# Sienna12321/MSHA--GNN

Measured on AMD Instinct MI355X. Metric: edges/sec GAT fwd+bwd @1 GPU; link-score pairs/sec; achieved HBM GB/s vs peak, higher is better.
Workload: dtype f32; 1 GPU; gat_layer_syn100k; nodes=100000, cols=100000, edges=2000000, in_features=128, heads=8, feat=16, parallelism=replicas1

## Files before the change

### msha--gnn_amd/csrc/edge_attention.hip

```cpp
#include <stdlib.h>

#include <cstdlib>

#include "common.h"
#include "edge_geo.h"

#ifndef COLS_EH
#define COLS_EH 1
#endif
#ifndef DE_SLOT_MIN_BYTES
#define DE_SLOT_MIN_BYTES (192ll << 20)
#endif
#ifndef COLS_WIDE_UG
#define COLS_WIDE_UG 4
#endif
#ifndef COLS_EPI_BUF
#define COLS_EPI_BUF 1
#endif
#ifndef COLS_NARROW_UG
#define COLS_NARROW_UG 8
#endif
#ifndef COLS_NG
#define COLS_NG 2
#endif

namespace msha {

template <int H, int F, typename T, int EPL>
__global__ void __launch_bounds__(256) edge_attn_fwd_kernel(
    const int32_t* __restrict__ rowptr, const int32_t* __restrict__ col,
    const uint8_t* __restrict__ rowflag, int64_t n_rows, const float* __restrict__ el,
    const float* __restrict__ er, const T* __restrict__ hc, float slope, Dropout dp,
    T* __restrict__ u, T* __restrict__ u_lo, float* __restrict__ lse, float* __restrict__ attd) {
  using G = Geo<H, F, T>;
  constexpr int CEL = EPL * G::CE;
  const int lane = lane_id();
  const int e_s = lane / H, h_s = lane % H;
  const int g_e = G::QPL == 1 ? lane / G::NQ : 0;
  const int64_t wave = ((int64_t)blockIdx.x * blockDim.x + threadIdx.x) >> 6;
  const int64_t nwaves = ((int64_t)gridDim.x * blockDim.x) >> 6;

  int64_t row = wave;
  if (row >= n_rows) return;
  int32_t start = rowptr[row], end = rowptr[row + 1];
  bool virt = rowflag != nullptr && rowflag[row] != 0;
  float elh = el[row * H + h_s];
  int32_t j0[EPL], j1[EPL];
#pragma unroll
  for (int t = 0; t < EPL; ++t) {
    const int32_t e0 = start + t * G::CE + e_s, e1 = e0 + CEL;
    j0[t] = e0 < end ? col[e0] : 0;
    j1[t] = e1 < end ? col[e1] : 0;
  }
  while (true) {
    const int64_t nrow = row + nwaves;
    const bool has_next = nrow < n_rows;
    const int32_t nstart = has_next ? rowptr[nrow] : 0;
    const int32_t nend = has_next ? rowptr[nrow + 1] : 0;
    float m = -INFINITY, l = 0.f;
    Pk<T> acc[G::QPL];
#pragma unroll
    for (int k = 0; k < G::QPL; ++k) acc[k] = pk_zero<T>();
    float erv[EPL];
#pragma unroll
    for (int t = 0; t < EPL; ++t)
      erv[t] = start + t * G::CE + e_s < end ? er[(int64_t)j0[t] * H + h_s] : 0.f;

    for (int32_t cs = start; cs < end; cs += CEL) {
      int32_t j[EPL], j2[EPL];
      float ern[EPL], sc[EPL];
      bool valid[EPL];
      float smax = -INFINITY;
#pragma unroll
      for (int t = 0; t < EPL; ++t) {
        const int32_t e = cs + t * G::CE + e_s;
        valid[t] = e < end;
        j[t] = j0[t];
        j2[t] = e + 2 * CEL < end ? col[e + 2 * CEL] : 0;
        ern[t] = e + CEL < end ? er[(int64_t)j1[t] * H + h_s] : 0.f;
        sc[t] = valid[t] ? (virt ? 0.f : lrelu(elh + erv[t], slope)) : -INFINITY;
        smax = fmaxf(smax, sc[t]);
      }
      const float mn = fmaxf(m, wave_xor_max<H>(smax));
      const float alpha = __expf(m - mn);
      float w[EPL], psum = 0.f;
#pragma unroll
      for (int t = 0; t < EPL; ++t) {
        const float pe = valid[t] ? __expf(sc[t] - mn) : 0.f;
        psum += pe;
        w[t] = valid[t] ? pe * dropout_factor(dp, (uint64_t)(cs + t * G::CE + e_s) * H + h_s)
                        : 0.f;
      }
      l = fmaf(l, alpha, wave_xor_sum<H>(psum));
      m = mn;
#pragma unroll
      for (int k = 0; k < G::QPL; ++k) {
        const int hd = quad_of<G>(lane, k) / G::QH;
        acc[k] = pk_scale(acc[k], __shfl(alpha, hd));
      }
      const int nvalid = min(CEL, (int)(end - cs));
#pragma unroll
      for (int g = 0; g < CEL; g += G::EPI) {
        if (g >= nvalid) break;
        const int t = g / G::CE;
        const int ei = g % G::CE + g_e;
        const int32_t jq = __shfl(j[t], ei * H);
// ... 479 lines not shown
        }
      }
    }
    if (G::EPI > 1) {
#pragma unroll
      for (int o = G::NQ; o < 64; o <<= 1) acc[0] = pk_xor_add(acc[0], o);
    }
#pragma unroll
    for (int k = 0; k < G::QPL; ++k) {
      if (g_e != 0) continue;
      const int q = quad_of<G>(lane, k);
      if (whole) {
        pk_store(out + (int64_t)jc * G::D + G::V * q, acc[k]);
      } else {
        float* dst = part + c * G::D + G::V * q;
#pragma unroll
        for (int i = 0; i < G::V; i += 4)
          *reinterpret_cast<float4*>(dst + i) =
              make_float4(acc[k].v[i], acc[k].v[i + 1], acc[k].v[i + 2], acc[k].v[i + 3]);
      }
    }
    if (HASX) {
      xacc = wave_xor_sum<H>(xacc);
      if (lane < H) (whole ? out_x + (int64_t)jc * H : part_x + c * H)[lane] = xacc;
    }
  }
}

constexpr int kCombineWaves = 16;

template <typename T>
__global__ void __launch_bounds__(1024) csc_combine_kernel(
    const int32_t* __restrict__ multi_col, const int32_t* __restrict__ multi_first,
    const int32_t* __restrict__ multi_count, int64_t n_multi, int D, int H,
    const float* __restrict__ part, const float* __restrict__ part_x, T* __restrict__ out,
    float* __restrict__ out_x) {
  __shared__ float red[kCombineWaves][256];
  const int W = D + (part_x != nullptr ? H : 0);
  const int64_t mi = blockIdx.x;
  const int e0 = blockIdx.y * 256;
  const int lane = threadIdx.x & 63, g = threadIdx.x >> 6;
  const int32_t jc = multi_col[mi], first = multi_first[mi], cnt = multi_count[mi];
  float acc[4] = {0.f, 0.f, 0.f, 0.f};
  auto ld = [&](int64_t c, int q) {
    const int e = e0 + lane + 64 * q;
    return e < D ? part[c * D + e] : (e < W ? part_x[c * H + (e - D)] : 0.f);
  };
  int k = g;
  for (; k + 3 * kCombineWaves < cnt; k += 4 * kCombineWaves) {
    float v[4][4];
#pragma unroll
    for (int u = 0; u < 4; ++u)
#pragma unroll
      for (int q = 0; q < 4; ++q) v[u][q] = ld(first + k + u * kCombineWaves, q);
#pragma unroll
    for (int u = 0; u < 4; ++u)
#pragma unroll
      for (int q = 0; q < 4; ++q) acc[q] += v[u][q];
  }
  for (; k < cnt; k += kCombineWaves) {
#pragma unroll
    for (int q = 0; q < 4; ++q) acc[q] += ld(first + k, q);
  }
#pragma unroll
  for (int q = 0; q < 4; ++q) red[g][lane + 64 * q] = acc[q];
  __syncthreads();
  for (int w = kCombineWaves / 2; w >= 1; w >>= 1) {
    if (g < w) {
#pragma unroll
      for (int q = 0; q < 4; ++q) red[g][lane + 64 * q] += red[g + w][lane + 64 * q];
    }
    __syncthreads();
  }
  if (g == 0) {
#pragma unroll
    for (int q = 0; q < 4; ++q) {
      const int e = e0 + lane + 64 * q;
      if (e < D) out[(int64_t)jc * D + e] = from_f32<T>(red[0][lane + 64 * q]);
      else if (e < W) out_x[(int64_t)jc * H + (e - D)] = red[0][lane + 64 * q];
    }
  }
}

#ifndef REC_PAD
#define REC_PAD 1
#endif
__host__ __device__ constexpr int rec_stride(int H) {
  int s = 1;
  while (s < 3 * H) s <<= 1;
  return REC_PAD ? s : 3 * H;
}
__host__ __device__ constexpr bool rec_has_flag(int H) { return rec_stride(H) > 3 * H; }

template <int H, int F, typename T, bool RT = false>
__global__ void __launch_bounds__(256) bwd_row_stats_kernel(
    int64_t n_rows, const float* __restrict__ el, const float* __restrict__ lse,
    const T* __restrict__ u, const T* __restrict__ u_lo, const T* __restrict__ dU,
    float* __restrict__ rec, const float* __restrict__ uc, const float* __restrict__ qc,
    const uint8_t* __restrict__ rowflag, float* __restrict__ d_el) {
  using G = Geo<H, F, T>;
  constexpr int UNR = G::QPL == 1 ? 4 : 1;
  constexpr int RPW = G::EPI * UNR;
  const int lane = lane_id();
  const int r_s = G::QPL == 1 ? lane / G::NQ : 0;
  const int64_t wave = ((int64_t)blockIdx.x * blockDim.x + threadIdx.x) >> 6;
  const int64_t nwaves = ((int64_t)gridDim.x * blockDim.x) >> 6;
  for (int64_t r0 = wave * RPW; r0 < n_rows; r0 += nwaves * RPW) {
    Pk<T> a[UNR][G::QPL], b[UNR][G::QPL];
    float4 c[UNR][G::QPL][RT ? G::V / 4 : 1];
    float elv[UNR][G::QPL], lsev[UNR][G::QPL], qcv[UNR][G::QPL];
    uint8_t fl[UNR];
    const bool lo = sizeof(T) == 2 && u_lo != nullptr;
#pragma unroll
    for (int g = 0; g < UNR; ++g) {
      const int64_t row = min(r0 + g * G::EPI + r_s, n_rows - 1);
#pragma unroll
      for (int k = 0; k < G::QPL; ++k) {
        const int q = quad_of<G>(lane, k);
        a[g][k] = pk_load(dU + row * G::D + G::V * q);
        b[g][k] = pk_load(u + row * G::D + G::V * q);
      }
#pragma unroll
      for (int k = 0; k < G::QPL; ++k) {
        const int q = quad_of<G>(lane, k);
        if (RT) {
#pragma unroll
          for (int v = 0; v < G::V / 4; ++v)
            c[g][k][v] = *reinterpret_cast<const float4*>(uc + row * G::D + G::V * q + 4 * v);
          qcv[g][k] = qc[row * H + q / G::QH];
        }
        elv[g][k] = el[row * H + q / G::QH];
        lsev[g][k] = lse[row * H + q / G::QH];
      }
      fl[g] = rowflag != nullptr ? rowflag[row] : (uint8_t)0;
    }
#pragma unroll
    for (int g = 0; g < UNR; ++g) {
      const int64_t row = r0 + g * G::EPI + r_s;
#pragma unroll
      for (int k = 0; k < G::QPL; ++k) {
        const int q = quad_of<G>(lane, k);
        float dot = pk_dot(a[g][k], b[g][k]);
        if (lo) {
          const int64_t rr = min(row, n_rows - 1);
          dot += pk_dot(a[g][k], pk_load(u_lo + rr * G::D + G::V * q));
        }
        const float dk = group_sum<G::QH>(dot);
        float dc = 0.f;
        if (RT) {
          float cv = 0.f;
#pragma unroll
          for (int v = G::V - 4; v >= 0; v -= 4) {
            const float4 c4 = c[g][k][v / 4];
            cv = fmaf(a[g][k].v[v + 3], c4.w, cv);
            cv = fmaf(a[g][k].v[v + 2], c4.z, cv);
            cv = fmaf(a[g][k].v[v + 1], c4.y, cv);
            cv = fmaf(a[g][k].v[v], c4.x, cv);
          }
          dc = group_sum<G::QH>(cv);
        }
        if (q % G::QH == 0 && row < n_rows) {
          const int h = q / G::QH;
          float* r = rec + row * rec_stride(H);
          r[h] = elv[g][k];
          r[H + h] = lsev[g][k];
          r[2 * H + h] = dk;
          const bool virt = fl[g] != 0;
          if (rec_has_flag(H) && h == 0) r[3 * H] = virt ? 1.f : 0.f;
          if (RT) d_el[row * H + h] = virt ? 0.f : fmaf(-dk, qcv[g][k], dc);
        }
      }
    }
  }
}

template <int H, int F, typename T, bool BUF, bool RSC = false>
__global__ void __launch_bounds__(256) bwd_cols_kernel(
    const int32_t* __restrict__ chunk_col, const int32_t* __restrict__ chunk_start,
    const int32_t* __restrict__ chunk_end, int64_t n_chunks, const int32_t* __restrict__ colptr,
    const int32_t* __restrict__ csc_row, const int32_t* __restrict__ csc_eid, int64_t n_rows,
    const uint8_t* __restrict__ rowflag, const float* __restrict__ rec,
    const float* __restrict__ er, const float* __restrict__ ar, const T* __restrict__ hc,
    const T* __restrict__ dU, float slope, Dropout dp, bool slot_de, float* __restrict__ de,
    T* __restrict__ d_hc, float* __restrict__ d_er, float* __restrict__ part,
    float* __restrict__ part_x) {
  using G = Geo<H, F, T>;
  const int lane = lane_id();
  const int e_s = lane / H, h_s = lane % H;
  const int g_e = G::QPL == 1 ? lane / G::NQ : 0;
  const int dsrc_k = (h_s * G::QH) / 64;
  const int dsrc_l = (h_s * G::QH) % 64;
  const int64_t wave = ((int64_t)blockIdx.x * blockDim.x + threadIdx.x) >> 6;
  const int64_t nwaves = ((int64_t)gridDim.x * blockDim.x) >> 6;

  int64_t c = wave;
  if (c >= n_chunks) return;
  int32_t jc = chunk_col[c], s0 = chunk_start[c], s1 = chunk_end[c];
  int32_t i0 = s0 + e_s < s1 ? csc_row[s0 + e_s] : 0;
  int32_t i1 = s0 + G::CE + e_s < s1 ? csc_row[s0 + G::CE + e_s] : 0;
  while (true) {
    const int64_t nc = c + nwaves;
    const bool has_next = nc < n_chunks;
    const int32_t njc = has_next ? chunk_col[nc] : 0;
    const int32_t ns0 = has_next ? chunk_start[nc] : 0;
    const int32_t ns1 = has_next ? chunk_end[nc] : 0;
    const bool whole = s0 == colptr[jc] && s1 == colptr[jc + 1];
    Pk<T> hcq[G::QPL], acc[G::QPL];
#pragma unroll
    for (int k = 0; k < G::QPL; ++k) {
      hcq[k] = pk_load(hc + (int64_t)jc * G::D + G::V * quad_of<G>(lane, k));
      acc[k] = pk_zero<T>();
    }
    float erh;
    if (RSC && G::QPL == 1) {
      const int q = lane % G::NQ;
      Pk<T> aq;
#pragma unroll
      for (int v = 0; v < G::V; ++v) aq.v[v] = ar[G::V * q + v];
      erh = __shfl(group_sum<G::QH>(pk_dot(hcq[0], aq)), h_s * G::QH);
    } else {
      erh = er[(int64_t)jc * H + h_s];
    }
    float xacc = 0.f;
    for (int32_t cs = s0; cs < s1; cs += G::CE) {
      const int32_t slot = cs + e_s;
      const bool valid = slot < s1;
      const int32_t i = i0;
      const int64_t eid = valid ? (int64_t)csc_eid[slot] : 0;
      float pre = 0.f, att = 0.f, dropf = 0.f, Dsi = 0.f;
      bool virt = false;
      if (valid) {
        const float* r = rec + (int64_t)i * rec_stride(H);
        virt = rowflag != nullptr && rowflag[i] != 0;
        pre = r[h_s] + erh;
        const float sv = virt ? 0.f : lrelu(pre, slope);
        att = __expf(sv - r[H + h_s]);
        Dsi = r[2 * H + h_s];
        dropf = dropout_factor(dp, (uint64_t)eid * H + h_s);
      }
      const float wv = att * dropf;
      const int nvalid = min(G::CE, (int)(s1 - cs));
      float gsum = 0.f;
      if constexpr (BUF && (G::EPI == 1 || COLS_EPI_BUF)) {
        constexpr int UG = G::EPI == 1 ? COLS_WIDE_UG : COLS_NARROW_UG;
        const rsrc_t r_dU = make_rsrc(dU, (uint32_t)(n_rows * G::D * sizeof(T)));
#pragma unroll
        for (int g0 = 0; g0 < G::CE; g0 += UG * G::EPI) {
          if (g0 >= nvalid) break;
          u32x4_t dl[UG][G::QPL];
#pragma unroll
          for (int u = 0; u < UG; ++u) {
            const int g = g0 + u * G::EPI;
            if (g >= G::CE) break;
            const int ei = g + g_e;
            const int32_t iq = __shfl(i, ei * H);
#pragma unroll
            for (int k = 0; k < G::QPL; ++k) {
              const int q = quad_of<G>(lane, k);
              const uint32_t off = ei < nvalid
                  ? (uint32_t)iq * (uint32_t)(G::D * sizeof(T)) + (uint32_t)(G::V * q * sizeof(T))
                  : kOOB;
              dl[u][k] = buf_b128(r_dU, off);
            }
          }
#pragma unroll
          for (int u = 0; u < UG; ++u) {
            const int g = g0 + u * G::EPI;
            if (g >= G::CE || g >= nvalid) break;
            const int ei = g + g_e;
            const bool mine = e_s >= g && e_s < g + G::EPI;
            const int srcl =
                G::QPL == 1 ? ((e_s - g) & (G::EPI - 1)) * G::NQ + h_s * G::QH : dsrc_l;
#pragma unroll
            for (int k = 0; k < G::QPL; ++k) {
              const int q = quad_of<G>(lane, k);
              const float wq = __shfl(wv, ei * H + q / G::QH);
              const Pk<T> dUi = pk_from_raw(dl[u][k], (T*)nullptr);
              acc[k] = pk_fma(wq, dUi, acc[k]);
              float t = pk_dot(dUi, hcq[k]);
              t = group_sum<G::QH>(t);
              const float cand = __shfl(t, srcl);
              if (mine && (G::QPL == 1 || k == dsrc_k)) gsum = cand;
            }
          }
        }
      } else {
#pragma unroll
      for (int g = 0; g < G::CE; g += G::EPI) {
        if (g >= nvalid) break;
        const int ei = g + g_e;
        const int32_t iq = __shfl(i, ei * H);
        const bool mine = e_s >= g && e_s < g + G::EPI;
        const int srcl = G::QPL == 1 ? ((e_s - g) & (G::EPI - 1)) * G::NQ + h_s * G::QH : dsrc_l;
#pragma unroll
        for (int k = 0; k < G::QPL; ++k) {
          const int q = quad_of<G>(lane, k);
          const float wq = __shfl(wv, ei * H + q / G::QH);
          float t = 0.f;
          if (ei < nvalid) {
            const Pk<T> dUi = pk_load(dU + (int64_t)iq * G::D + G::V * q);
            acc[k] = pk_fma(wq, dUi, acc[k]);
            t = pk_dot(dUi, hcq[k]);
          }
          t = group_sum<G::QH>(t);
          const float cand = __shfl(t, srcl);
          if (mine && (G::QPL == 1 || k == dsrc_k)) gsum = cand;
        }
      }
      }
      const int32_t sl2 = slot + 2 * G::CE;
      const int32_t i2 = sl2 < s1 ? csc_row[sl2] : 0;
      if (valid) {
        const float ds = att * (gsum * dropf - Dsi);
        const float dev = virt ? 0.f : ds * (pre > 0.f ? 1.f : slope);
        if (de != nullptr) de[(slot_de ? (int64_t)slot : eid) * H + h_s] = dev;
        xacc += dev;
      }
      i0 = i1;
      i1 = i2;
    }
    if (has_next) {
      const int32_t a0 = ns0 + e_s, a1 = ns0 + G::CE + e_s;
      i0 = a0 < ns1 ? csc_row[a0] : 0;
      i1 = a1 < ns1 ? csc_row[a1] : 0;
    }
    if (G::EPI > 1) {
#pragma unroll
      for (int o = G::NQ; o < 64; o <<= 1) acc[0] = pk_xor_add(acc[0], o);
    }
#pragma unroll
    for (int k = 0; k < G::QPL; ++k) {
      if (g_e != 0) continue;
      const int q = quad_of<G>(lane, k);
      if (whole) {
        pk_store(d_hc + (int64_t)jc * G::D + G::V * q, acc[k]);
      } else {
        float* dst = part + c * G::D + G::V * q;
#pragma unroll
        for (int v = 0; v < G::V; v += 4)
          *reinterpret_cast<float4*>(dst + v) =
              make_float4(acc[k].v[v], acc[k].v[v + 1], acc[k].v[v + 2], acc[k].v[v + 3]);
      }
    }
    xacc = wave_xor_sum<H>(xacc);
    if (lane < H) (whole ? d_er + (int64_t)jc * H : part_x + c * H)[lane] = xacc;
    if (!has_next) break;
    c = nc;
    jc = njc;
    s0 = ns0;
    s1 = ns1;
  }
}

template <int H, int F, typename T, bool RSC = false>
__global__ void __launch_bounds__(256) bwd_cols_eh_kernel(
    const int32_t* __restrict__ chunk_col, const int32_t* __restrict__ chunk_start,
    const int32_t* __restrict__ chunk_end, int64_t n_chunks, const int32_t* __restrict__ colptr,
    const int32_t* __restrict__ csc_row, const int32_t* __restrict__ csc_eid, int64_t n_edges,
    const uint8_t* __restrict__ rowflag, int64_t n_rows, const float* __restrict__ rec,
    const float* __restrict__ er, const float* __restrict__ ar, const T* __restrict__ hc,
    const T* __restrict__ dU, float slope, Dropout dp, bool slot_de, float* __restrict__ de,
    T* __restrict__ d_hc, float* __restrict__ d_er, float* __restrict__ part,
    float* __restrict__ part_x) {
  using G = Geo<H, F, T>;
  constexpr int NV = G::QH;
  constexpr int NG = COLS_NG;
  const int lane = lane_id();
  const int e_s = lane / H, h_s = lane % H;
  const int64_t wave = ((int64_t)blockIdx.x * blockDim.x + threadIdx.x) >> 6;
  const int64_t nwaves = ((int64_t)gridDim.x * blockDim.x) >> 6;
  const rsrc_t r_row = make_rsrc(csc_row, (uint32_t)(n_edges * 4));
  const rsrc_t r_eid = make_rsrc(csc_eid, (uint32_t)(n_edges * 4));
  const rsrc_t r_flag = make_rsrc(rowflag, (uint32_t)n_rows);
  const rsrc_t r_rec = make_rsrc(rec, (uint32_t)(n_rows * 4 * rec_stride(H)));
  const rsrc_t r_dU = make_rsrc(dU, (uint32_t)(n_rows * G::D * sizeof(T)));
  const rsrc_t r_de = make_rsrc(de, (uint32_t)(n_edges * 4 * H));
  const uint32_t h_off = h_s * F * sizeof(T);
  const bool need_eid = dp.active || (de != nullptr && !slot_de);

  int64_t c = wave;
  if (c >= n_chunks) return;
  int32_t jc = chunk_col[c], s0 = chunk_start[c], s1 = chunk_end[c];
  int32_t ii[NG];
#pragma unroll
  for (int g = 0; g < NG; ++g) {
    const int32_t a = s0 + g * G::CE + e_s;
    ii[g] = buf_i32(r_row, a < s1 ? (uint32_t)a * 4u : kOOB);
  }
  while (true) {
    const int64_t nc = c + nwaves;
    const bool has_next = nc < n_chunks;
    const int32_t njc = has_next ? chunk_col[nc] : 0;
    const int32_t ns0 = has_next ? chunk_start[nc] : 0;
    const int32_t ns1 = has_next ? chunk_end[nc] : 0;
    const bool whole = s0 == colptr[jc] && s1 == colptr[jc + 1];
    Pk<T> hcv[NV], acc[NV];
#pragma unroll
    for (int k = 0; k < NV; ++k) {
      hcv[k] = pk_load(hc + (int64_t)jc * G::D + h_s * F + G::V * k);
      acc[k] = pk_zero<T>();
    }
    const float er_tab = RSC ? 0.f : er[(int64_t)jc * H + h_s];
    float xacc = 0.f;
    for (int32_t cs = s0; cs < s1; cs += NG * G::CE) {
      Pk<T> dUv[NG][NV];
      int32_t eid[NG];
      float r_el[NG], r_lse[NG], Dsi[NG];
      uint32_t vflag[NG];
#pragma unroll
      for (int g = 0; g < NG; ++g) {
        const bool valid = cs + g * G::CE + e_s < s1;
        const uint32_t row_off = valid ? (uint32_t)ii[g] * (G::D * sizeof(T)) + h_off : kOOB;
#pragma unroll
        for (int k = 0; k < NV; ++k)
          dUv[g][k] = pk_load_buf(r_dU, row_off + (valid ? k * 16u : 0u), (T*)nullptr);
        eid[g] = buf_i32(r_eid, valid && need_eid ? (uint32_t)(cs + g * G::CE + e_s) * 4u : kOOB);
        const uint32_t rec_off = valid ? (uint32_t)ii[g] * (4u * rec_stride(H)) + h_s * 4u : kOOB;
        r_el[g] = buf_f32(r_rec, rec_off);
        r_lse[g] = buf_f32(r_rec, valid ? rec_off + 4u * H : kOOB);
        Dsi[g] = buf_f32(r_rec, valid ? rec_off + 8u * H : kOOB);
        if constexpr (rec_has_flag(H))
          vflag[g] = __float_as_uint(buf_f32(r_rec, valid ? rec_off - h_s * 4u + 12u * H : kOOB));
        else
          vflag[g] = buf_u8(r_flag, valid ? (uint32_t)ii[g] : kOOB);
      }
#pragma unroll
      for (int g = 0; g < NG; ++g) {
        const int32_t a = cs + (NG + g) * G::CE + e_s;
        ii[g] = buf_i32(r_row, a < s1 ? (uint32_t)a * 4u : kOOB);
      }
      float erh = er_tab;
      if (RSC) {
        Pk<T> hv[NV];
#pragma unroll
        for (int k = 0; k < NV; ++k) {
          hv[k] = hcv[k];
#pragma unroll
          for (int v = 0; v < G::V; ++v) asm volatile("" : "+v"(hv[k].v[v]));
        }
        erh = head_score<NV>(hv, ar + h_s * F);
      }
#pragma unroll
      for (int g = 0; g < NG; ++g) {
        const int32_t slot = cs + g * G::CE + e_s;
        const bool valid = slot < s1;
        const bool virt = vflag[g] != 0;
        const float pre = r_el[g] + erh;
        const float sv = virt ? 0.f : lrelu(pre, slope);
        const float att = __expf(sv - r_lse[g]);
        const float dropf = dropout_factor(dp, (uint64_t)eid[g] * H + h_s);
        const float wv = valid ? att * dropf : 0.f;
        float d[NV];
#pragma unroll
        for (int k = 0; k < NV; ++k) {
          d[k] = pk_dot(dUv[g][k], hcv[k]);
          acc[k] = pk_fma(wv, dUv[g][k], acc[k]);
        }
#pragma unroll
        for (int o = 1; o < NV; o <<= 1)
#pragma unroll
          for (int k = 0; k < NV; k += 2 * o) d[k] = d[k] + d[k + o];
        const float ds = att * (d[0] * dropf - Dsi[g]);
        const float dev = virt ? 0.f : ds * (pre > 0.f ? 1.f : slope);
#ifndef DIAG_NO_DE
        const uint32_t at = slot_de ? (uint32_t)slot : (uint32_t)eid[g];
        buf_store_f32(r_de, valid ? at * (4u * H) + h_s * 4u : kOOB, dev);
#endif
        xacc += valid ? dev : 0.f;
      }
    }
#pragma unroll
    for (int g = 0; g < NG; ++g) {
      const int32_t a = ns0 + g * G::CE + e_s;
      ii[g] = buf_i32(r_row, a < ns1 ? (uint32_t)a * 4u : kOOB);
    }
#pragma unroll
    for (int k = 0; k < NV; ++k)
#pragma unroll
      for (int o = H; o < 64; o <<= 1) acc[k] = pk_xor_add(acc[k], o);
    if (e_s == 0) {
#pragma unroll
      for (int k = 0; k < NV; ++k) {
        if (whole) {
          pk_store(d_hc + (int64_t)jc * G::D + h_s * F + G::V * k, acc[k]);
        } else {
          float* dst = part + c * G::D + h_s * F + G::V * k;
#pragma unroll
          for (int v = 0; v < G::V; v += 4)
            *reinterpret_cast<float4*>(dst + v) =
                make_float4(acc[k].v[v], acc[k].v[v + 1], acc[k].v[v + 2], acc[k].v[v + 3]);
        }
      }
    }
    xacc = wave_xor_sum<H>(xacc);
    if (lane < H) (whole ? d_er + (int64_t)jc * H : part_x + c * H)[lane] = xacc;
    if (!has_next) break;
    c = nc;
    jc = njc;
    s0 = ns0;
    s1 = ns1;
  }
}

template <int H>
__global__ void __launch_bounds__(256) bwd_row_sum_kernel(
    const int32_t* __restrict__ rowptr, int64_t n_rows, const float* __restrict__ de,
    const int32_t* __restrict__ slot_of, float* __restrict__ d_el) {
  constexpr int CE = 64 / H;
  const int lane = lane_id();
  const int r_s = lane / H, h_s = lane % H;
  const int64_t wave = ((int64_t)blockIdx.x * blockDim.x + threadIdx.x) >> 6;
  const int64_t nwaves = ((int64_t)gridDim.x * blockDim.x) >> 6;
  for (int64_t r0 = wave * CE; r0 < n_rows; r0 += nwaves * CE) {
    const int64_t row = r0 + r_s;
    if (row >= n_rows) continue;
    const int32_t start = rowptr[row], end = rowptr[row + 1];
    float p[CE];
#pragma unroll
    for (int k = 0; k < CE; ++k) p[k] = 0.f;
    for (int32_t cs = start; cs < end; cs += CE) {
      float v[CE];
      int32_t at[CE];
#pragma unroll
      for (int k = 0; k < CE; ++k)
        at[k] = slot_of == nullptr ? cs + k : (cs + k < end ? slot_of[cs + k] : 0);
#pragma unroll
      for (int k = 0; k < CE; ++k)
        v[k] = cs + k < end ? de[(int64_t)at[k] * H + h_s] : 0.f;
#pragma unroll
      for (int k = 0; k < CE; ++k)
        if (cs + k < end) p[k] += v[k];
    }
#pragma unroll
    for (int o = 1; o < CE; o <<= 1) {
#pragma unroll
      for (int k = 0; k < CE; ++k)
        if ((k & o) == 0 && (k & (2 * o - 1)) == 0) p[k] = p[k] + p[k + o];
    }
    d_el[row * H + h_s] = p[0];
  }
}

static bool shape_supported(int H, int F) {
#define X(h, f) if (H == h && F == f) return true;
  MSHA_FOR_EACH_SHAPE(X)
#undef X
  return false;
}

static int env_int(const char* name, int def) {
// ... 200 lines not shown
}

extern "C" size_t msha_csc_aggregate_workspace_size(const msha_graph* g, int32_t heads,
                                                    int32_t feat) {
  if (g == nullptr || heads <= 0 || feat <= 0) return 0;
  const size_t per = (size_t)heads * (size_t)feat + (size_t)heads;
  return (size_t)g->n_chunks * per * sizeof(float) + 256;
}

template <typename T>
static void launch_csc(const msha_graph* g, int heads, int feat, const float* w, const float* x,
                       int ld, const void* table, void* out, float* out_x, float* part,
                       float* part_x, hipStream_t s) {
#define X(h, f)                                                                                 \
  if (heads == h && feat == f) {                                                                \
    if constexpr (f % Pk<T>::V == 0) {                                                          \
      if (x)                                                                                    \
        hipLaunchKernelGGL((csc_aggregate_kernel<h, f, T, true>), wave_grid(g->n_chunks),       \
                           dim3(256), 0, s, g->chunk_col, g->chunk_start, g->chunk_end,         \
                           g->n_chunks, g->colptr, g->csc_row, g->csc_eid, w, x, ld,            \
                           (const T*)table, (T*)out, out_x, part, part_x);                      \
      else                                                                                      \
        hipLaunchKernelGGL((csc_aggregate_kernel<h, f, T, false>), wave_grid(g->n_chunks),      \
                           dim3(256), 0, s, g->chunk_col, g->chunk_start, g->chunk_end,         \
                           g->n_chunks, g->colptr, g->csc_row, g->csc_eid, w, x, ld,            \
                           (const T*)table, (T*)out, out_x, part, part_x);                      \
    }                                                                                           \
  }
  MSHA_FOR_EACH_SHAPE(X)
#undef X
  if (g->n_multi > 0) {
    const int64_t D = (int64_t)heads * feat;
    const int64_t W = D + (x ? heads : 0);
    hipLaunchKernelGGL(csc_combine_kernel<T>, dim3(g->n_multi, (W + 255) / 256),
                       dim3(64 * kCombineWaves), 0, s, g->multi_col, g->multi_first,
                       g->multi_count, g->n_multi, (int)D, heads, part, x ? part_x : nullptr,
                       (T*)out, out_x);
  }
}

extern "C" int msha_csc_aggregate(const msha_graph* g, int32_t heads, int32_t feat,
                                  int32_t dtype, const float* w, const float* x, int32_t edge_ld,
                                  const void* table, void* out, float* out_x, void* ws,
                                  size_t ws_bytes, msha_stream_t stream) {
  if (int rc = check_graph(g, true)) return rc;
  MSHA_ARG_CHECK(w && table && out, "csc_aggregate: null pointer");
  MSHA_ARG_CHECK(x == nullptr || out_x != nullptr, "csc_aggregate: x needs out_x");
  if (!shape_supported(heads, feat) || !dtype_ok(dtype, feat))
    return fail(MSHA_ERR_UNSUPPORTED, "csc_aggregate: unsupported (heads, feat, dtype)");
  const int64_t D = (int64_t)heads * feat;
  float* part = nullptr;
  float* part_x = nullptr;
  if (g->n_multi > 0) {
    MSHA_ARG_CHECK(ws != nullptr && ws_bytes >= msha_csc_aggregate_workspace_size(g, heads, feat),
                   "csc_aggregate: workspace too small");
    part = (float*)ws;
    part_x = part + g->n_chunks * D;
  }
  hipStream_t s = (hipStream_t)stream;
  const int ld = edge_ld > 0 ? edge_ld : heads;
  MSHA_ARG_CHECK(ld >= heads, "csc_aggregate: edge_ld < heads");
  if (dtype == MSHA_DTYPE_BF16)
    launch_csc<bf16_t>(g, heads, feat, w, x, ld, table, out, out_x, part, part_x, s);
  else
    launch_csc<float>(g, heads, feat, w, x, ld, table, out, out_x, part, part_x, s);
  return check_launch("csc_aggregate");
}

extern "C" size_t msha_edge_attention_bwd_fused_workspace_size(const msha_graph* g,
                                                               int32_t heads, int32_t feat) {
  if (g == nullptr || heads <= 0 || feat <= 0) return 0;
  const size_t rec = ((size_t)g->n_rows * rec_stride(heads) * sizeof(float) + 255) & ~(size_t)255;
  return rec + msha_csc_aggregate_workspace_size(g, heads, feat);
}

template <typename T>
static void launch_bwd_fused(const msha_graph* g, int heads, int feat, const float* el,
                             const float* er, const float* ar, const void* hc, const float* lse, const void* u,
                             const void* u_lo, const void* dU, float neg_slope, const Dropout& dp, float* d_el,
                             float* d_er, void* d_hc, float* de, float* rec, float* part,
                             float* part_x, const float* uc, const float* qc, hipStream_t s) {
  const bool rt = uc != nullptr;
  if (rt) de = nullptr;
  const int64_t lim = (int64_t)1 << 31;
  const bool slot_de = g->csr_slot != nullptr && g->n_edges * 4 * (int64_t)heads >= DE_SLOT_MIN_BYTES;
  const char* nobuf = getenv("MSHA_COLS_NOBUF");
  const bool buf_ok = !(nobuf != nullptr && *nobuf == '1') &&
                      g->n_rows * (int64_t)heads * feat * (int64_t)sizeof(T) < lim &&
                      g->n_edges * 4 * (int64_t)heads < lim && g->n_rows * 4 * rec_stride(heads) < lim;
#define X(h, f)                                                                                \
  if (heads == h && feat == f) {                                                               \
    if constexpr (f % Pk<T>::V == 0) {                                                         \
      auto row_stats = rt ? bwd_row_stats_kernel<h, f, T, true>                                \
                          : bwd_row_stats_kernel<h, f, T, false>;                              \
      hipLaunchKernelGGL(row_stats,                                                            \
                         wave_grid(g->n_rows / 8 + 1), dim3(256), 0, s, g->n_rows, el, lse,   \
                         (const T*)u, (const T*)u_lo, (const T*)dU, rec, uc, qc, g->rowflag,  \
                         d_el);                                                                \
      if (f * sizeof(T) <= 64 && COLS_EH && buf_ok)                                            \
        hipLaunchKernelGGL((ar != nullptr ? bwd_cols_eh_kernel<h, f, T, true>                 \
                                           : bwd_cols_eh_kernel<h, f, T, false>),               \
                           wave_grid(g->n_chunks), dim3(256), 0,                                \
                           s, g->chunk_col, g->chunk_start, g->chunk_end, g->n_chunks,         \
                           g->colptr, g->csc_row, g->csc_eid, g->n_edges, g->rowflag,          \
                           g->n_rows, rec, er, ar, (const T*)hc, (const T*)dU, neg_slope, dp,  \
                           slot_de, de,                                                        \
                           (T*)d_hc, d_er, part, part_x);                                      \
      else                                                                                     \
      {                                                                                        \
        auto kern = ar != nullptr                                                              \
            ? (buf_ok ? bwd_cols_kernel<h, f, T, true, true> : bwd_cols_kernel<h, f, T, false, true>) \
            : (buf_ok ? bwd_cols_kernel<h, f, T, true> : bwd_cols_kernel<h, f, T, false>);     \
        hipLaunchKernelGGL(kern, wave_grid(g->n_chunks), dim3(256), 0,                         \
                           s, g->chunk_col, g->chunk_start, g->chunk_end, g->n_chunks,         \
                           g->colptr, g->csc_row, g->csc_eid, g->n_rows, g->rowflag, rec, er,  \
                           ar, (const T*)hc, (const T*)dU, neg_slope, dp, slot_de,             \
                           de, (T*)d_hc, d_er,                                                 \
                           part, part_x);                                                      \
      }                                                                                        \
      if (!rt)                                                                                 \
        hipLaunchKernelGGL((bwd_row_sum_kernel<h>), wave_grid(g->n_rows), dim3(256), 0, s,     \
                           g->rowptr, g->n_rows, de, slot_de ? g->csr_slot : nullptr, d_el);  \
    }                                                                                          \
  }
  MSHA_FOR_EACH_SHAPE(X)
#undef X
  if (g->n_multi > 0) {
    const int64_t D = (int64_t)heads * feat;
    hipLaunchKernelGGL(csc_combine_kernel<T>, dim3(g->n_multi, (D + heads + 255) / 256),
                       dim3(64 * kCombineWaves), 0, s, g->multi_col, g->multi_first,
                       g->multi_count, g->n_multi, (int)D, heads, part, part_x, (T*)d_hc, d_er);
  }
}

extern "C" int msha_edge_attention_bwd_fused(const msha_graph* g, int32_t heads, int32_t feat,
                                             int32_t dtype, const float* el, const float* er,
                                             const void* hc, const float* lse, const void* u,
                                             const void* u_lo, const void* dU, float neg_slope,
                                             float drop_p,
                                             uint64_t seed, uint64_t offset, float* d_el,
                                             float* d_er, void* d_hc, float* de, void* ws,
                                             size_t ws_bytes, msha_stream_t stream) {
  return msha_edge_attention_bwd_fused_ex(g, heads, feat, dtype, el, er, hc, lse, u, u_lo, dU,
                                          neg_slope, drop_p, seed, offset, nullptr, nullptr,
                                          d_el, d_er, d_hc, de, ws, ws_bytes, stream);
}

extern "C" int msha_edge_attention_bwd_fused_ex(
    const msha_graph* g, int32_t heads, int32_t feat, int32_t dtype, const float* el,
    const float* er, const void* hc, const float* lse, const void* u, const void* u_lo,
    const void* dU, float neg_slope, float drop_p, uint64_t seed, uint64_t offset,
    const float* uc, const float* qc, float* d_el, float* d_er, void* d_hc, float* de, void* ws,
    size_t ws_bytes, msha_stream_t stream) {
  if (int rc = check_graph(g, true)) return rc;
  MSHA_ARG_CHECK(el && er && hc && lse && u && dU && d_el && d_er && d_hc,
                 "edge_attention_bwd_fused: null pointer");
  MSHA_ARG_CHECK((uc == nullptr) == (qc == nullptr), "edge_attention_bwd_fused: uc and qc go together");
  MSHA_ARG_CHECK(g->n_edges == 0 || ((de || uc) && g->csc_eid),
                 "edge_attention_bwd_fused: needs de scratch (or row terms) and csc_eid");
  MSHA_ARG_CHECK(drop_p >= 0.f && drop_p <= 1.f, "edge_attention_bwd_fused: p must be in [0,1]");
  if (!shape_supported(heads, feat) || !dtype_ok(dtype, feat))
    return fail(MSHA_ERR_UNSUPPORTED, "edge_attention_bwd_fused: unsupported (heads, feat, dtype)");
  MSHA_ARG_CHECK(ws != nullptr &&
                     ws_bytes >= msha_edge_attention_bwd_fused_workspace_size(g, heads, feat),
                 "edge_attention_bwd_fused: workspace too small");
  const int64_t D = (int64_t)heads * feat;
  float* rec = (float*)ws;
  const size_t rec_bytes = ((size_t)g->n_rows * rec_stride(heads) * sizeof(float) + 255) & ~(size_t)255;
  float* part = (float*)((char*)ws + rec_bytes);
  float* part_x = part + g->n_chunks * D;
  hipStream_t s = (hipStream_t)stream;
  const Dropout dp = make_dropout(drop_p, seed, offset, s);
  if (dtype == MSHA_DTYPE_BF16)
    launch_bwd_fused<bf16_t>(g, heads, feat, el, er, nullptr, hc, lse, u, u_lo, dU, neg_slope, dp,
                             d_el, d_er, d_hc, de, rec, part, part_x, uc, qc, s);
  else
    launch_bwd_fused<float>(g, heads, feat, el, er, nullptr, hc, lse, u, nullptr, dU, neg_slope, dp,
                            d_el, d_er, d_hc, de, rec, part, part_x, uc, qc, s);
  return check_launch("edge_attention_bwd_fused");
}

extern "C" int msha_edge_attention_row_scores_supported(const msha_graph* g, int32_t heads,
                                                        int32_t feat, int32_t dtype) {
  if (g == nullptr || !shape_supported(heads, feat) || !dtype_ok(dtype, feat)) return 0;
  return fwd_bat_ok(g, heads, feat, dtype) ? 1 : 0;
}

#ifndef RS_BF16_MIN_BYTES
#define RS_BF16_MIN_BYTES 0ll
#endif
extern "C" int msha_edge_attention_row_scores_preferred(const msha_graph* g, int32_t heads,
                                                        int32_t feat, int32_t dtype) {
  if (!msha_edge_attention_row_scores_supported(g, heads, feat, dtype)) return 0;
  const int knob = env_int("MSHA_ROW_SCORES", -1);
  if (knob >= 0) return knob != 0;
  if (dtype == MSHA_DTYPE_F32) return 1;
  return g->n_cols * 4 * (int64_t)heads >= RS_BF16_MIN_BYTES ? 1 : 0;
}

extern "C" int msha_edge_attention_fwd_rs(const msha_graph* g, int32_t heads, int32_t feat,
                                          int32_t dtype, const float* el, const float* ar,
                                          const void* hc, float neg_slope, float drop_p,
                                          uint64_t seed, uint64_t offset, void* u, void* u_lo,
                                          float* lse, float* uc, float* qc,
                                          msha_stream_t stream) {
  if (int rc = check_graph(g, false)) return rc;
  MSHA_ARG_CHECK(el && ar && hc && u && lse, "edge_attention_fwd_rs: null pointer");
  MSHA_ARG_CHECK(drop_p >= 0.f && drop_p <= 1.f, "edge_attention_fwd_rs: p must be in [0,1]");
  MSHA_ARG_CHECK((uc == nullptr) == (qc == nullptr), "edge_attention_fwd_rs: uc and qc go together");
  MSHA_ARG_CHECK(((uintptr_t)ar & 15) == 0, "edge_attention_fwd_rs: a_r must be 16-byte aligned");
  if (!msha_edge_attention_row_scores_supported(g, heads, feat, dtype))
    return fail(MSHA_ERR_UNSUPPORTED, "edge_attention_fwd_rs: unsupported (heads, feat, dtype, sizes)");
  hipStream_t s = (hipStream_t)stream;
  const Dropout dp = make_dropout(drop_p, seed, offset, s);
  const bool short_rows = g->n_edges <= (int64_t)FWD_SHORT_DEG * g->n_rows;
  if (!launch_fwd_gl(g, heads, feat, dtype, el, nullptr, ar, hc, neg_slope, dp, u, u_lo, lse,
                     nullptr, uc, qc, short_rows, fwd_grid(g), s))
    return fail(MSHA_ERR_UNSUPPORTED, "edge_attention_fwd_rs: shape not compiled");
  return check_launch("edge_attention_fwd_rs");
}

extern "C" int msha_edge_attention_bwd_fused_rs(
    const msha_graph* g, int32_t heads, int32_t feat, int32_t dtype, const float* el,
    const float* ar, const void* hc, const float* lse, const void* u, const void* u_lo,
    const void* dU, float neg_slope, float drop_p, uint64_t seed, uint64_t offset,
    const float* uc, const float* qc, float* d_el, float* d_er, void* d_hc, float* de, void* ws,
    size_t ws_bytes, msha_stream_t stream) {
  if (int rc = check_graph(g, true)) return rc;
  MSHA_ARG_CHECK(el && ar && hc && lse && u && dU && d_el && d_er && d_hc,
                 "edge_attention_bwd_fused_rs: null pointer");
  MSHA_ARG_CHECK((uc == nullptr) == (qc == nullptr), "edge_attention_bwd_fused_rs: uc and qc go together");
  MSHA_ARG_CHECK(g->n_edges == 0 || ((de || uc) && g->csc_eid),
                 "edge_attention_bwd_fused_rs: needs de scratch (or row terms) and csc_eid");
  MSHA_ARG_CHECK(drop_p >= 0.f && drop_p <= 1.f, "edge_attention_bwd_fused_rs: p must be in [0,1]");
  MSHA_ARG_CHECK(((uintptr_t)ar & 15) == 0, "edge_attention_bwd_fused_rs: a_r must be 16-byte aligned");
  if (!msha_edge_attention_row_scores_supported(g, heads, feat, dtype))
    return fail(MSHA_ERR_UNSUPPORTED, "edge_attention_bwd_fused_rs: unsupported (heads, feat, dtype, sizes)");
  MSHA_ARG_CHECK(ws != nullptr &&
                     ws_bytes >= msha_edge_attention_bwd_fused_workspace_size(g, heads, feat),
                 "edge_attention_bwd_fused_rs: workspace too small");
  const int64_t D = (int64_t)heads * feat;
  float* rec = (float*)ws;
  const size_t rec_bytes = ((size_t)g->n_rows * rec_stride(heads) * sizeof(float) + 255) & ~(size_t)255;
  float* part = (float*)((char*)ws + rec_bytes);
  float* part_x = part + g->n_chunks * D;
  hipStream_t s = (hipStream_t)stream;
  const Dropout dp = make_dropout(drop_p, seed, offset, s);
  if (dtype == MSHA_DTYPE_BF16)
    launch_bwd_fused<bf16_t>(g, heads, feat, el, nullptr, ar, hc, lse, u, u_lo, dU, neg_slope, dp,
                             d_el, d_er, d_hc, de, rec, part, part_x, uc, qc, s);
  else
    launch_bwd_fused<float>(g, heads, feat, el, nullptr, ar, hc, lse, u, nullptr, dU, neg_slope, dp,
                            d_el, d_er, d_hc, de, rec, part, part_x, uc, qc, s);
  return check_launch("edge_attention_bwd_fused_rs");
}
```

Before: 4.719 billion edges/s.

## Interleave per-head row records as float4 and add lean cols path without dropout

Changes the per-row backward record from a head-major layout (el, lse, D blocks plus a flag) to one float4 per (row, head) holding el, lse, D and the virtual flag. The column kernels then fetch it with a single 16-byte load instead of three or four scalar loads plus a separate rowflag byte read. It also adds a LEAN template variant, used when dropout is inactive and no per-edge de output is needed, which skips the csc_eid gather, the dropout hash and the de store. A sched_barrier is inserted after the loads, and a 16-byte workspace alignment check is added.

```diff
diff --git a/msha--gnn_amd/csrc/edge_attention.hip b/msha--gnn_amd/csrc/edge_attention.hip
--- a/msha--gnn_amd/csrc/edge_attention.hip
+++ b/msha--gnn_amd/csrc/edge_attention.hip
@@ -22,6 +22,9 @@
 #endif
 #ifndef COLS_NG
 #define COLS_NG 2
+#endif
+#ifndef COLS_LEAN
+#define COLS_LEAN 1
 #endif
 
 namespace msha {
@@ -667,15 +670,8 @@
   }
 }
 
-#ifndef REC_PAD
-#define REC_PAD 1
-#endif
-__host__ __device__ constexpr int rec_stride(int H) {
-  int s = 1;
-  while (s < 3 * H) s <<= 1;
-  return REC_PAD ? s : 3 * H;
-}
-__host__ __device__ constexpr bool rec_has_flag(int H) { return rec_stride(H) > 3 * H; }
+__host__ __device__ constexpr int rec_stride(int H) { return 4 * H; }
+static_assert(rec_stride(8) * sizeof(float) == 128, "H = 8: the record is one 128-B line");
 
 template <int H, int F, typename T, bool RT = false>
 __global__ void __launch_bounds__(256) bwd_row_stats_kernel(
@@ -746,12 +742,9 @@
         }
         if (q % G::QH == 0 && row < n_rows) {
           const int h = q / G::QH;
-          float* r = rec + row * rec_stride(H);
-          r[h] = elv[g][k];
-          r[H + h] = lsev[g][k];
-          r[2 * H + h] = dk;
           const bool virt = fl[g] != 0;
-          if (rec_has_flag(H) && h == 0) r[3 * H] = virt ? 1.f : 0.f;
+          *reinterpret_cast<float4*>(rec + (row * H + h) * 4) =
+              make_float4(elv[g][k], lsev[g][k], dk, virt ? 1.f : 0.f);
           if (RT) d_el[row * H + h] = virt ? 0.f : fmaf(-dk, qcv[g][k], dc);
         }
       }
@@ -759,12 +752,12 @@
   }
 }
 
-template <int H, int F, typename T, bool BUF, bool RSC = false>
+template <int H, int F, typename T, bool BUF, bool RSC = false, bool LEAN = false>
 __global__ void __launch_bounds__(256) bwd_cols_kernel(
     const int32_t* __restrict__ chunk_col, const int32_t* __restrict__ chunk_start,
     const int32_t* __restrict__ chunk_end, int64_t n_chunks, const int32_t* __restrict__ colptr,
     const int32_t* __restrict__ csc_row, const int32_t* __restrict__ csc_eid, int64_t n_rows,
-    const uint8_t* __restrict__ rowflag, const float* __restrict__ rec,
+    const float* __restrict__ rec,
     const float* __restrict__ er, const float* __restrict__ ar, const T* __restrict__ hc,
     const T* __restrict__ dU, float slope, Dropout dp, bool slot_de, float* __restrict__ de,
     T* __restrict__ d_hc, float* __restrict__ d_er, float* __restrict__ part,
@@ -811,17 +804,17 @@
       const int32_t slot = cs + e_s;
       const bool valid = slot < s1;
       const int32_t i = i0;
-      const int64_t eid = valid ? (int64_t)csc_eid[slot] : 0;
+      const int64_t eid = !LEAN && valid ? (int64_t)csc_eid[slot] : 0;
       float pre = 0.f, att = 0.f, dropf = 0.f, Dsi = 0.f;
       bool virt = false;
       if (valid) {
-        const float* r = rec + (int64_t)i * rec_stride(H);
-        virt = rowflag != nullptr && rowflag[i] != 0;
-        pre = r[h_s] + erh;
+        const float4 r = *reinterpret_cast<const float4*>(rec + ((int64_t)i * H + h_s) * 4);
+        virt = r.w != 0.f;
+        pre = r.x + erh;
         const float sv = virt ? 0.f : lrelu(pre, slope);
-        att = __expf(sv - r[H + h_s]);
-        Dsi = r[2 * H + h_s];
-        dropf = dropout_factor(dp, (uint64_t)eid * H + h_s);
+        att = __expf(sv - r.y);
+        Dsi = r.z;
+        dropf = LEAN ? 1.f : dropout_factor(dp, (uint64_t)eid * H + h_s);
       }
       const float wv = att * dropf;
       const int nvalid = min(G::CE, (int)(s1 - cs));
@@ -898,7 +891,7 @@
       if (valid) {
         const float ds = att * (gsum * dropf - Dsi);
         const float dev = virt ? 0.f : ds * (pre > 0.f ? 1.f : slope);
-        if (de != nullptr) de[(slot_de ? (int64_t)slot : eid) * H + h_s] = dev;
+        if (!LEAN && de != nullptr) de[(slot_de ? (int64_t)slot : eid) * H + h_s] = dev;
         xacc += dev;
       }
       i0 = i1;
@@ -937,12 +930,12 @@
   }
 }
 
-template <int H, int F, typename T, bool RSC = false>
+template <int H, int F, typename T, bool RSC = false, bool LEAN = false>
 __global__ void __launch_bounds__(256) bwd_cols_eh_kernel(
     const int32_t* __restrict__ chunk_col, const int32_t* __restrict__ chunk_start,
     const int32_t* __restrict__ chunk_end, int64_t n_chunks, const int32_t* __restrict__ colptr,
     const int32_t* __restrict__ csc_row, const int32_t* __restrict__ csc_eid, int64_t n_edges,
-    const uint8_t* __restrict__ rowflag, int64_t n_rows, const float* __restrict__ rec,
+    int64_t n_rows, const float* __restrict__ rec,
     const float* __restrict__ er, const float* __restrict__ ar, const T* __restrict__ hc,
     const T* __restrict__ dU, float slope, Dropout dp, bool slot_de, float* __restrict__ de,
     T* __restrict__ d_hc, float* __restrict__ d_er, float* __restrict__ part,
@@ -956,7 +949,6 @@
   const int64_t nwaves = ((int64_t)gridDim.x * blockDim.x) >> 6;
   const rsrc_t r_row = make_rsrc(csc_row, (uint32_t)(n_edges * 4));
   const rsrc_t r_eid = make_rsrc(csc_eid, (uint32_t)(n_edges * 4));
-  const rsrc_t r_flag = make_rsrc(rowflag, (uint32_t)n_rows);
   const rsrc_t r_rec = make_rsrc(rec, (uint32_t)(n_rows * 4 * rec_stride(H)));
   const rsrc_t r_dU = make_rsrc(dU, (uint32_t)(n_rows * G::D * sizeof(T)));
   const rsrc_t r_de = make_rsrc(de, (uint32_t)(n_edges * 4 * H));
@@ -990,8 +982,7 @@
     for (int32_t cs = s0; cs < s1; cs += NG * G::CE) {
       Pk<T> dUv[NG][NV];
       int32_t eid[NG];
-      float r_el[NG], r_lse[NG], Dsi[NG];
-      uint32_t vflag[NG];
+      u32x4_t rp[NG];
 #pragma unroll
       for (int g = 0; g < NG; ++g) {
         const bool valid = cs + g * G::CE + e_s < s1;
@@ -999,21 +990,18 @@
 #pragma unroll
         for (int k = 0; k < NV; ++k)
           dUv[g][k] = pk_load_buf(r_dU, row_off + (valid ? k * 16u : 0u), (T*)nullptr);
-        eid[g] = buf_i32(r_eid, valid && need_eid ? (uint32_t)(cs + g * G::CE + e_s) * 4u : kOOB);
-        const uint32_t rec_off = valid ? (uint32_t)ii[g] * (4u * rec_stride(H)) + h_s * 4u : kOOB;
-        r_el[g] = buf_f32(r_rec, rec_off);
-        r_lse[g] = buf_f32(r_rec, valid ? rec_off + 4u * H : kOOB);
-        Dsi[g] = buf_f32(r_rec, valid ? rec_off + 8u * H : kOOB);
-        if constexpr (rec_has_flag(H))
-          vflag[g] = __float_as_uint(buf_f32(r_rec, valid ? rec_off - h_s * 4u + 12u * H : kOOB));
+        if constexpr (LEAN)
+          eid[g] = 0;
         else
-          vflag[g] = buf_u8(r_flag, valid ? (uint32_t)ii[g] : kOOB);
+          eid[g] = buf_i32(r_eid, valid && need_eid ? (uint32_t)(cs + g * G::CE + e_s) * 4u : kOOB);
+        rp[g] = buf_b128(r_rec, valid ? (uint32_t)ii[g] * (16u * H) + h_s * 16u : kOOB);
       }
 #pragma unroll
       for (int g = 0; g < NG; ++g) {
         const int32_t a = cs + (NG + g) * G::CE + e_s;
         ii[g] = buf_i32(r_row, a < s1 ? (uint32_t)a * 4u : kOOB);
       }
+      __builtin_amdgcn_sched_barrier(0);
       float erh = er_tab;
       if (RSC) {
         Pk<T> hv[NV];
@@ -1029,11 +1017,12 @@
       for (int g = 0; g < NG; ++g) {
         const int32_t slot = cs + g * G::CE + e_s;
         const bool valid = slot < s1;
-        const bool virt = vflag[g] != 0;
-        const float pre = r_el[g] + erh;
+        const bool virt = rp[g].w != 0;
+        const float pre = __uint_as_float(rp[g].x) + erh;
         const float sv = virt ? 0.f : lrelu(pre, slope);
-        const float att = __expf(sv - r_lse[g]);
-        const float dropf = dropout_factor(dp, (uint64_t)eid[g] * H + h_s);
+        const float att = __expf(sv - __uint_as_float(rp[g].y));
+        const float Dsi = __uint_as_float(rp[g].z);
+        const float dropf = LEAN ? 1.f : dropout_factor(dp, (uint64_t)eid[g] * H + h_s);
         const float wv = valid ? att * dropf : 0.f;
         float d[NV];
 #pragma unroll
@@ -1045,12 +1034,12 @@
         for (int o = 1; o < NV; o <<= 1)
 #pragma unroll
           for (int k = 0; k < NV; k += 2 * o) d[k] = d[k] + d[k + o];
-        const float ds = att * (d[0] * dropf - Dsi[g]);
+        const float ds = att * (d[0] * dropf - Dsi);
         const float dev = virt ? 0.f : ds * (pre > 0.f ? 1.f : slope);
-#ifndef DIAG_NO_DE
-        const uint32_t at = slot_de ? (uint32_t)slot : (uint32_t)eid[g];
-        buf_store_f32(r_de, valid ? at * (4u * H) + h_s * 4u : kOOB, dev);
-#endif
+        if constexpr (!LEAN) {
+          const uint32_t at = slot_de ? (uint32_t)slot : (uint32_t)eid[g];
+          buf_store_f32(r_de, valid ? at * (4u * H) + h_s * 4u : kOOB, dev);
+        }
         xacc += valid ? dev : 0.f;
       }
     }
@@ -1417,6 +1406,7 @@
                              float* part_x, const float* uc, const float* qc, hipStream_t s) {
   const bool rt = uc != nullptr;
   if (rt) de = nullptr;
+  const bool lean = COLS_LEAN && de == nullptr && !dp.active;
   const int64_t lim = (int64_t)1 << 31;
   const bool slot_de = g->csr_slot != nullptr && g->n_edges * 4 * (int64_t)heads >= DE_SLOT_MIN_BYTES;
   const char* nobuf = getenv("MSHA_COLS_NOBUF");
@@ -1432,23 +1422,29 @@
                          wave_grid(g->n_rows / 8 + 1), dim3(256), 0, s, g->n_rows, el, lse,   \
                          (const T*)u, (const T*)u_lo, (const T*)dU, rec, uc, qc, g->rowflag,  \
                          d_el);                                                                \
-      if (f * sizeof(T) <= 64 && COLS_EH && buf_ok)                                            \
-        hipLaunchKernelGGL((ar != nullptr ? bwd_cols_eh_kernel<h, f, T, true>                 \
-                                           : bwd_cols_eh_kernel<h, f, T, false>),               \
-                           wave_grid(g->n_chunks), dim3(256), 0,                                \
+      if (f * sizeof(T) <= 64 && COLS_EH && buf_ok) {                                          \
+        auto kern = ar != nullptr                                                              \
+            ? (lean ? bwd_cols_eh_kernel<h, f, T, true, true> : bwd_cols_eh_kernel<h, f, T, true>)   \
+            : (lean ? bwd_cols_eh_kernel<h, f, T, false, true> : bwd_cols_eh_kernel<h, f, T, false>); \
+        hipLaunchKernelGGL(kern, wave_grid(g->n_chunks), dim3(256), 0,                         \
                            s, g->chunk_col, g->chunk_start, g->chunk_end, g->n_chunks,         \
-                           g->colptr, g->csc_row, g->csc_eid, g->n_edges, g->rowflag,          \
+                           g->colptr, g->csc_row, g->csc_eid, g->n_edges,                      \
                            g->n_rows, rec, er, ar, (const T*)hc, (const T*)dU, neg_slope, dp,  \
                            slot_de, de,                                                        \
                            (T*)d_hc, d_er, part, part_x);                                      \
-      else                                                                                     \
-      {                                                                                        \
+      } else {                                                                                 \
         auto kern = ar != nullptr                                                              \
-            ? (buf_ok ? bwd_cols_kernel<h, f, T, true, true> : bwd_cols_kernel<h, f, T, false, true>) \
-            : (buf_ok ? bwd_cols_kernel<h, f, T, true> : bwd_cols_kernel<h, f, T, false>);     \
+            ? (buf_ok ? (lean ? bwd_cols_kernel<h, f, T, true, true, true>                     \
+                              : bwd_cols_kernel<h, f, T, true, true>)                          \
+                      : (lean ? bwd_cols_kernel<h, f, T, false, true, true>                    \
+                              : bwd_cols_kernel<h, f, T, false, true>))                        \
+            : (buf_ok ? (lean ? bwd_cols_kernel<h, f, T, true, false, true>                    \
+                              : bwd_cols_kernel<h, f, T, true>)                                \
+                      : (lean ? bwd_cols_kernel<h, f, T, false, false, true>                   \
+                              : bwd_cols_kernel<h, f, T, false>));                             \
         hipLaunchKernelGGL(kern, wave_grid(g->n_chunks), dim3(256), 0,                         \
                            s, g->chunk_col, g->chunk_start, g->chunk_end, g->n_chunks,         \
-                           g->colptr, g->csc_row, g->csc_eid, g->n_rows, g->rowflag, rec, er,  \
+                           g->colptr, g->csc_row, g->csc_eid, g->n_rows, rec, er,              \
                            ar, (const T*)hc, (const T*)dU, neg_slope, dp, slot_de,             \
                            de, (T*)d_hc, d_er,                                                 \
                            part, part_x);                                                      \
@@ -1499,6 +1495,7 @@
   MSHA_ARG_CHECK(ws != nullptr &&
                      ws_bytes >= msha_edge_attention_bwd_fused_workspace_size(g, heads, feat),
                  "edge_attention_bwd_fused: workspace too small");
+  MSHA_ARG_CHECK(((uintptr_t)ws & 15) == 0, "edge_attention_bwd_fused: workspace must be 16-byte aligned");
   const int64_t D = (int64_t)heads * feat;
   float* rec = (float*)ws;
   const size_t rec_bytes = ((size_t)g->n_rows * rec_stride(heads) * sizeof(float) + 255) & ~(size_t)255;
@@ -1574,6 +1571,7 @@
   MSHA_ARG_CHECK(ws != nullptr &&
                      ws_bytes >= msha_edge_attention_bwd_fused_workspace_size(g, heads, feat),
                  "edge_attention_bwd_fused_rs: workspace too small");
+  MSHA_ARG_CHECK(((uintptr_t)ws & 15) == 0, "edge_attention_bwd_fused_rs: workspace must be 16-byte aligned");
   const int64_t D = (int64_t)heads * feat;
   float* rec = (float*)ws;
   const size_t rec_bytes = ((size_t)g->n_rows * rec_stride(heads) * sizeof(float) + 255) & ~(size_t)255;
```

Measured after the change: 4.724 billion edges/s (median of 3 runs). Within noise of the previous version (+0.1%).
